# tkoolen/Parametron.jl

Hardware: AMD Instinct MI355X
Metric: QP re-evaluations/sec (Q,q,C,d rebuild) at n=4096 (higher is better)
Workload: dtype f64; 1 GPU; C2 dense least-squares QP: n=4096 vars, A 4096x4096, m=512 equality rows, fp64; canonical Q,q,const + C,d MOI triplets; n=4096, r=4096, m=512, objective_mode=canonical, instances_per_gpu=1, parallelism=single GPU, replay=tape

## Files before the change

parametron.jl_amd/csrc/gram_mid.hip:

```cpp
#include "gram_common.h"

#ifndef PMT_MID_WPS
#define PMT_MID_WPS 1
#endif
#ifndef PMT_MID_G
#define PMT_MID_G 256
#endif
#ifndef PMT_MID_MAXWG
#define PMT_MID_MAXWG 2304
#endif
#ifndef PMT_MID_D
#define PMT_MID_D 2
#endif
#ifndef PMT_MID_GROUP_US
#define PMT_MID_GROUP_US 1.15
#endif
#ifndef PMT_MID_TAIL_US
#define PMT_MID_TAIL_US 0.95
#endif
#ifndef PMT_MID_XCD
#define PMT_MID_XCD 1
#endif
#ifndef PMT_MID_SUPER
#define PMT_MID_SUPER 1
#endif
#ifndef PMT_MID_PERSIST
#define PMT_MID_PERSIST 1
#endif
#ifndef PMT_MID_SB
#define PMT_MID_SB 8
#endif
#ifndef PMT_MID_FB
#define PMT_MID_FB 4
#endif
#ifndef PMT_MID_SCHED
#define PMT_MID_SCHED 2
#endif
#ifndef PMT_MID_ABL
#define PMT_MID_ABL 0
#endif
#ifndef PMT_MID_FORMAL
#if defined(__HIP_DEVICE_COMPILE__) && !defined(__gfx950__) && !defined(__gfx942__)
#define PMT_MID_FORMAL 1
#else
#define PMT_MID_FORMAL 0
#endif
#endif

#ifdef PMT_MID_TRACE
__device__ unsigned long long g_mid_trace[1024 * 8];
#define MID_STAMP(k) do { if (threadIdx.x == 0 && blockIdx.x < 1024) g_mid_trace[blockIdx.x * 8 + (k)] = wall_clock64(); } while (0)
extern "C" int pmt_mid_trace_read(unsigned long long *host) {
    return hipMemcpyFromSymbol(host, HIP_SYMBOL(g_mid_trace), sizeof(unsigned long long) * 1024 * 8) == hipSuccess ? 0 : 1;
}
#else
#define MID_STAMP(k) do { } while (0)
#endif

namespace pmt {

constexpr int MT = 64;
constexpr int MACC = 64;
constexpr int MPART = MACC * 64;
constexpr int MSTRIDE = MPART + MT + 8;
constexpr int MPITCH = MT + 1;
constexpr int MFG = 8;
constexpr int MCNT = 16;
constexpr int MQBUF = 4 * 2048;
constexpr int MFLAG = MQBUF + 4 * MT;
constexpr int MMAPS = MFLAG + 8;
constexpr int MSH = MMAPS + 2 * MT;

struct MidArgs {
    const double *A; int64_t lda, rows, cols;
    const double *b; int sign;
    const int64_t *xvar; const int64_t *varmap; int moi;
    QT *out_quad; double *out_csc; double alpha; LT *out_lin; double *out_const;
    int nb;
    int n_off, s_off, s_diag;
    int gpc_off, gpc_diag;
    int n_tail, s_tail, gpc_tail;
    double *ws;
    unsigned *counters;
    int xcd;
    int persist, total;
    unsigned *tickets;
};

struct MidPlan { int nb, n_off, s_off, s_diag, gpc_off, gpc_diag, n_tail, s_tail, gpc_tail, wgs; };

static double mid_fold_us(int count) { return 0.5 + 2.6 * (double)cdiv(count, PMT_MID_FB); }

static MidPlan mid_plan(int64_t rows, int64_t cols) {
    MidPlan p;
    p.nb = (int)cdiv(cols, MT);
    p.n_off = p.nb * (p.nb - 1) / 2;
    const int ngroups = (int)std::max<int64_t>(1, cdiv(rows, 8));
    const int maxs = std::max(1, ngroups / 4);
    auto sd = [&](int s) { return std::min(maxs, std::max(1, (5 * s + 7) / 8)); };
    int best = 1;
    double best_t = 1e300;
    for (int s = 1; s <= std::min(maxs, 64); ++s) {
        const int64_t wgs = (int64_t)p.n_off * s + (int64_t)p.nb * sd(s);
        if (s > 1 && wgs > PMT_MID_MAXWG) break;
        const double it_off = (double)cdiv(cdiv(ngroups, s), 4), it_diag = 0.69 * (double)cdiv(cdiv(ngroups, sd(s)), 4);
        const double fold = s <= 1 ? 0.0 : s <= MFG ? mid_fold_us(s) : mid_fold_us(MFG) + 1.5 + mid_fold_us((int)cdiv(s, MFG));
        const double t = (double)cdiv(wgs, PMT_MID_G) * (PMT_MID_GROUP_US * (p.n_off ? std::max(it_off, it_diag) : it_diag) + 5.0 + (s > 1 ? 1.0 : 0.0)) +
                         fold * (1.0 + (double)(p.n_off + p.nb) / PMT_MID_G);
        if (t < best_t) { best_t = t; best = s; }
    }
    int s = best;
#ifdef PMT_TUNING
    if (const char *e = getenv("PMT_MID_S")) { const int v = atoi(e); if (v > 0) s = std::min(v, maxs); }
#endif
    int sdiag = sd(s), ntail = 0, stail = 1;
    if (p.n_off + p.nb > PMT_MID_G) {
        auto wg_us = [&](int c, double w) { return PMT_MID_TAIL_US * w * (double)cdiv(cdiv(ngroups, c), 4) + 5.0 + (c > 1 ? 1.0 : 0.0); };
        const int rem = p.n_off % PMT_MID_G;
        int ct = 1;
        double tail_off = 0.0;
        if (rem) {
            tail_off = 1e300;
            for (int c = 1; c <= std::min(maxs, MFG); ++c) {
                const double t = (double)cdiv((int64_t)rem * c, PMT_MID_G) * wg_us(c, 1.0) + (c > 1 ? mid_fold_us(c) : 0.0);
                if (t < tail_off) { tail_off = t; ct = c; }
            }
        }
        const int last = rem ? (int)(((int64_t)rem * ct) % PMT_MID_G) : 0, free_cus = last ? PMT_MID_G - last : 0;
        const double t_last = rem ? wg_us(ct, 1.0) : wg_us(1, 1.0);
        int cd = 1;
        double tail_diag = 1e300;
        for (int c = 1; c <= std::min(maxs, MFG); ++c) {
            const double t_d = wg_us(c, 0.69);
            const int64_t inside = (int64_t)free_cus * (int64_t)(t_last / t_d);
            const int64_t left = std::max<int64_t>(0, (int64_t)p.nb * c - inside);
            const double t = (double)cdiv(left, PMT_MID_G) * t_d + (c > 1 ? mid_fold_us(c) : 0.0);
            if (t < tail_diag) { tail_diag = t; cd = c; }
        }
        const double t1 = (double)(p.n_off / PMT_MID_G) * wg_us(1, 1.0) + tail_off + tail_diag;
        if (s == 1 || t1 * (PMT_MID_GROUP_US / PMT_MID_TAIL_US) < best_t) { s = 1; sdiag = cd; ntail = ct > 1 ? rem : 0; stail = ct > 1 ? ct : 1; }
    }
#ifdef PMT_TUNING
    if (const char *e = getenv("PMT_MID_TAIL")) { if (atoi(e) == 0) { ntail = 0; stail = 1; } }
#endif
    p.gpc_off = (int)cdiv(ngroups, s);
    p.s_off = (int)cdiv(ngroups, p.gpc_off);
    p.gpc_diag = (int)cdiv(ngroups, sdiag);
    p.s_diag = (int)cdiv(ngroups, p.gpc_diag);
    p.n_tail = ntail;
    p.gpc_tail = (int)cdiv(ngroups, stail);
    p.s_tail = ntail ? (int)cdiv(ngroups, p.gpc_tail) : 1;
    if (p.s_tail <= 1) { p.n_tail = 0; p.s_tail = 1; p.gpc_tail = ngroups; }
    p.wgs = (p.n_off - p.n_tail) * p.s_off + p.n_tail * p.s_tail + p.nb * p.s_diag + 1;
    return p;
}

template <bool DIAG, bool FAST>
__device__ __forceinline__ void mid_load(const MidArgs &g, int64_t row0, int lane, int64_t cj0, int64_t ck0, const unsigned (&voff)[DIAG ? 4 : 8],
                                         f64x2 (&buf)[DIAG ? 4 : 8], f64x2 &cb) {
    constexpr int NG = DIAG ? 4 : 8;
    const int lm = lane & 15, lk = lane >> 4;
    if (FAST) {
        const char *base = reinterpret_cast<const char *>(g.A + row0);
#pragma unroll
        for (int t = 0; t < NG; ++t) buf[t] = *reinterpret_cast<const f64x2 *>(base + voff[t]);
        cb.x = 0.0; cb.y = 0.0;
        if (DIAG && g.b) cb = *reinterpret_cast<const f64x2 *>(g.b + row0 + 2 * lk);
        return;
    }
    const int64_t row = row0 + 2 * lk;
    const bool r0 = row < g.rows, r1 = row + 1 < g.rows;
#pragma unroll
    for (int t = 0; t < NG; ++t) {
        const int64_t col = (t < 4 ? cj0 : ck0) + 16 * (t & 3) + lm;
        const bool cv = col < g.cols;
        const bool v0 = cv && r0, v1 = cv && r1;
        const double *p0 = g.A + (v0 ? col * g.lda + row : 0), *p1 = g.A + (v1 ? col * g.lda + row + 1 : 0);
        const double x = *p0, y = *p1;
        buf[t].x = v0 ? x : 0.0;
        buf[t].y = v1 ? y : 0.0;
    }
    cb.x = 0.0; cb.y = 0.0;
    if (DIAG && g.b) {
        const double x = g.b[r0 ? row : 0], y = g.b[r1 ? row + 1 : 0];
        cb.x = r0 ? x : 0.0;
        cb.y = r1 ? y : 0.0;
    }
}

template <bool DIAG>
__device__ __forceinline__ void mid_compute(double *__restrict__ rot, const f64x2 (&buf)[DIAG ? 4 : 8], const f64x2 &cb, int sign, int lane,
                                            double (&acc)[MACC], double (&qacc)[4]) {
    constexpr int BO = DIAG ? 0 : 4;
    const int lm = lane & 15, lrow = lane & 48;
#pragma unroll
    for (int t = 0; t < (PMT_MID_ABL == 5 || PMT_MID_ABL == 6 ? 0 : 4); ++t) *reinterpret_cast<f64x2 *>(rot + (t * 64 + lane) * 2) = buf[BO + t];
    f64x2 bv[4][4];
#pragma unroll
    for (int c = 0; c < 4; ++c) {
        bv[c][0] = buf[BO + c];
#pragma unroll
        for (int r = 1; r < 4; ++r) {
            if (PMT_MID_ABL == 5 || PMT_MID_ABL == 6) { bv[c][r] = buf[BO + (PMT_MID_ABL == 6 ? 0 : c)]; continue; }
            bv[c][r] = *reinterpret_cast<const f64x2 *>(rot + (c * 64 + lrow + ((lm + 4 * r) & 15)) * 2);
        }
    }
#if PMT_MID_SCHED
    __builtin_amdgcn_sched_barrier(0);
#endif
    constexpr int NC = PMT_MID_ABL == 1 ? 0 : 4;
#pragma unroll
    for (int c = 0; c < NC; ++c)
#pragma unroll
        for (int tm = 0; tm < (DIAG ? c + 1 : 4); ++tm) {
            const int a = (tm * 4 + c) * 4;
            acc[a] = __builtin_amdgcn_mfma_f64_4x4x4f64(buf[tm].x, bv[c][0].x, acc[a], 0, 0, 0);
        }
#pragma unroll
    for (int c = 0; c < NC; ++c)
#pragma unroll
        for (int tm = 0; tm < (DIAG ? c + 1 : 4); ++tm) {
            const int a = (tm * 4 + c) * 4;
            acc[a] = __builtin_amdgcn_mfma_f64_4x4x4f64(buf[tm].y, bv[c][0].y, acc[a], 0, 0, 0);
        }
#if PMT_MID_SCHED
    __builtin_amdgcn_sched_barrier(0);
#endif
#pragma unroll
    for (int c = 0; c < NC; ++c) {
#pragma unroll
        for (int r = 1; r < 4; ++r)
#pragma unroll
            for (int tm = 0; tm < (DIAG ? c + 1 : 4); ++tm) {
                const int a = (tm * 4 + c) * 4 + r;
                acc[a] = __builtin_amdgcn_mfma_f64_4x4x4f64(buf[tm].x, bv[c][r].x, acc[a], 0, 0, 0);
            }
#pragma unroll
        for (int r = 1; r < 4; ++r)
#pragma unroll
            for (int tm = 0; tm < (DIAG ? c + 1 : 4); ++tm) {
                const int a = (tm * 4 + c) * 4 + r;
                acc[a] = __builtin_amdgcn_mfma_f64_4x4x4f64(buf[tm].y, bv[c][r].y, acc[a], 0, 0, 0);
            }
    }
    if (DIAG) {
        const double c0 = signed_const(cb.x, sign), c1 = signed_const(cb.y, sign);
#pragma unroll
        for (int t = 0; t < 4; ++t) qacc[t] = __builtin_amdgcn_mfma_f64_4x4x4f64(buf[t].x, c0, qacc[t], 0, 0, 0);
#pragma unroll
        for (int t = 0; t < 4; ++t) qacc[t] = __builtin_amdgcn_mfma_f64_4x4x4f64(buf[t].y, c1, qacc[t], 0, 0, 0);
    }
}

#define MID_SB() __builtin_amdgcn_sched_barrier(0)
template <bool DIAG>
__device__ __forceinline__ void mid_step(const MidArgs &g, double *__restrict__ rot, int64_t next_row0, unsigned (&voff)[DIAG ? 4 : 8],
                                         f64x2 (&buf)[DIAG ? 4 : 8], f64x2 &cb, int sign, int lane, double (&acc)[MACC], double (&qacc)[4]) {
    constexpr int BO = DIAG ? 0 : 4;
    const int lm = lane & 15, lrow = lane & 48, lk = lane >> 4;
    const char *base = reinterpret_cast<const char *>(g.A + next_row0);
    auto reload = [&](int t) {
        asm volatile("" : "+v"(voff[t]));
        buf[t] = *reinterpret_cast<const f64x2 *>(base + voff[t]);
    };
    f64x2 bv[4][4];
#pragma unroll
    for (int c = 0; c < 4; ++c) bv[c][0] = buf[BO + c];
    auto lds_op = [&](int i) {
        if (i < 4) *reinterpret_cast<f64x2 *>(rot + (i * 64 + lane) * 2) = buf[BO + i];
        else {
            const int c = (i - 4) / 3, r = 1 + (i - 4) % 3;
            bv[c][r] = *reinterpret_cast<const f64x2 *>(rot + (c * 64 + lrow + ((lm + 4 * r) & 15)) * 2);
        }
    };
    MID_SB();
    int k = 0;
#pragma unroll
    for (int pass = 0; pass < 2; ++pass)
#pragma unroll
        for (int c = 0; c < 4; ++c)
#pragma unroll
            for (int tm = 0; tm < (DIAG ? c + 1 : 4); ++tm) {
                const int a = (tm * 4 + c) * 4;
                acc[a] = __builtin_amdgcn_mfma_f64_4x4x4f64(pass ? buf[tm].y : buf[tm].x, pass ? bv[c][0].y : bv[c][0].x, acc[a], 0, 0, 0);
                if (k < 16) { MID_SB(); lds_op(k); MID_SB(); }
                ++k;
            }
    if (DIAG) {
        const double c0 = signed_const(cb.x, sign), c1 = signed_const(cb.y, sign);
#pragma unroll
        for (int t = 0; t < 4; ++t) qacc[t] = __builtin_amdgcn_mfma_f64_4x4x4f64(buf[t].x, c0, qacc[t], 0, 0, 0);
#pragma unroll
        for (int t = 0; t < 4; ++t) qacc[t] = __builtin_amdgcn_mfma_f64_4x4x4f64(buf[t].y, c1, qacc[t], 0, 0, 0);
        MID_SB();
        cb = *reinterpret_cast<const f64x2 *>((g.b ? g.b : g.A) + next_row0 + 2 * lk);
    }
    MID_SB();
    int nb = 0;
#pragma unroll
    for (int tm = 0; tm < 4; ++tm) {
#pragma unroll
        for (int pass = 0; pass < 2; ++pass)
#pragma unroll
            for (int c = (DIAG ? tm : 0); c < 4; ++c)
#pragma unroll
                for (int r = 1; r < 4; ++r) {
                    const int a = (tm * 4 + c) * 4 + r;
                    acc[a] = __builtin_amdgcn_mfma_f64_4x4x4f64(pass ? buf[tm].y : buf[tm].x, pass ? bv[c][r].y : bv[c][r].x, acc[a], 0, 0, 0);
                    if (!DIAG && nb < 4) { MID_SB(); reload(4 + nb); MID_SB(); ++nb; }
                }
        MID_SB();
        reload(tm);
        MID_SB();
    }
}

__host__ __device__ constexpr bool mid_used(bool diag, int a) { return !diag || (a >> 4) <= ((a >> 2) & 3); }

__device__ __forceinline__ void mid_pos(int lane, int a, int &row, int &col) {
    const int i = lane >> 4, b = (lane >> 2) & 3, j = lane & 3;
    row = 16 * (a >> 4) + 4 * b + i;
    col = 16 * ((a >> 2) & 3) + 4 * ((b + (a & 3)) & 3) + j;
}

__device__ __forceinline__ void mid_maps(const MidArgs &g, double *sh, int tid, int jb, int kb) {
    u64 *cmap = reinterpret_cast<u64 *>(sh + MMAPS);
    if (tid >= 2 * MT || (!g.out_quad && jb != kb)) return;
    const int64_t i = (tid < MT ? (int64_t)kb * MT + tid : (int64_t)jb * MT + tid - MT);
    const int64_t v = i < g.cols ? g.xvar[i] : 1;
    cmap[tid] = (u64)(g.moi ? map_var(g.varmap, v) : v);
}

__device__ __forceinline__ void mid_epilogue(const MidArgs &g, double *sh, int tid, int jb, int kb) {
    const int wave = tid >> 6, lane = tid & 63;
    const int64_t n = g.cols, j0 = (int64_t)jb * MT, k0 = (int64_t)kb * MT;
    double *tile = sh;
    const double *qfin = sh + MT * MPITCH;
    const u64 *cmap = reinterpret_cast<const u64 *>(sh + MMAPS);
    const u64 *rmap = cmap + MT;
    if (g.out_csc) {
        const int64_t j = j0 + lane;
#pragma unroll 4
        for (int col = wave; col < MT; col += 4) {
            const int64_t k = k0 + col;
            double c = tile[lane * MPITCH + col];
            if (g.moi || j != k) c = 2 * c;
            if (k < n && j <= k) g.out_csc[k * (k + 1) / 2 + j] = g.alpha * c;
        }
    }
    if (g.out_quad) {
        u64 *out = reinterpret_cast<u64 *>(g.out_quad);
        u64 *desc = reinterpret_cast<u64 *>(sh + MT * MPITCH + MT);
        if (tid < MT) {
            const int64_t j = j0 + tid;
            const int64_t kstart = j > k0 ? j : k0;
            const int64_t kend = (k0 + MT < n) ? k0 + MT : n;
            const int64_t nterms = (j < n && kend > kstart) ? kend - kstart : 0;
            desc[2 * tid] = (u64)(j * n - (j * (j - 1)) / 2 + (kstart - j)) * 3;
            desc[2 * tid + 1] = (u64)nterms | (u64)(kstart - k0) << 16 | (u64)(kstart == j ? 1 : 0) << 24;
        }
        __syncthreads();
        const bool moi = g.moi != 0;
        const int uwave = __builtin_amdgcn_readfirstlane(wave);
#pragma unroll 4
        for (int i = 0; i < MT / 4; ++i) {
            const int row = 4 * i + uwave;
            const u64 w0 = desc[2 * row], info = desc[2 * row + 1];
            const int nterms = (int)(info & 0xffff), coff = (int)((info >> 16) & 0xff);
            const bool dg = ((info >> 24) & 1) != 0;
            double c = tile[row * MPITCH + coff + lane];
            const u64 m = cmap[(coff + lane) & (MT - 1)], rv = rmap[row];
            if (moi || !(dg && lane == 0)) c = 2 * c;
            if (lane < nterms) {
                u64 *d = out + w0 + 3 * lane;
                d[0] = (u64)__double_as_longlong(c);
                d[1] = rv;
                d[2] = m;
            }
        }
    }
    if (jb == kb && tid < MT) {
        const int64_t j = j0 + tid;
        if (j < n) {
            LT t;
            t.coeff = 2 * qfin[tid];
            t.var = (int64_t)rmap[tid];
            g.out_lin[j] = t;
        }
    }
}

__device__ __forceinline__ void mid_constant(const MidArgs &g, double *sh, int tid) {
    const int wave = tid >> 6, lane = tid & 63;
    double s0 = 0.0, s1 = 0.0;
    if (g.b && g.sign) {
        for (int64_t i = tid; i < g.rows; i += 512) { const double c = signed_const(g.b[i], g.sign); s0 = s0 + c * c; }
        for (int64_t i = tid + 256; i < g.rows; i += 512) { const double c = signed_const(g.b[i], g.sign); s1 = s1 + c * c; }
    }
#pragma unroll
    for (int off = 32; off > 0; off >>= 1) { s0 = s0 + __shfl_down(s0, off, 64); s1 = s1 + __shfl_down(s1, off, 64); }
    if (lane == 0) { sh[wave] = s0; sh[4 + wave] = s1; }
    __syncthreads();
    if (tid == 0) {
        double v = sh[0];
#pragma unroll
        for (int w = 1; w < 8; ++w) v = v + sh[w];
        *g.out_const = v;
    }
}

__device__ __forceinline__ void mid_put(double *p, double v) {
#if PMT_MID_FORMAL
    *p = v;
#else
    __hip_atomic_store(p, v, __ATOMIC_RELAXED, __HIP_MEMORY_SCOPE_AGENT);
#endif
}
__device__ __forceinline__ double mid_get(const double *p) {
#if PMT_MID_FORMAL
    return *p;
#else
    return __hip_atomic_load(p, __ATOMIC_RELAXED, __HIP_MEMORY_SCOPE_AGENT);
#endif
}

template <bool DIAG, int W>
__device__ __forceinline__ void mid_tail(const MidArgs &g, double *sh, int lane, double (&acc)[MACC], const double (&qacc)[4], int nchunk, double *w) {
    constexpr int KEEP1 = (W >> 1) * 32, GIVE1 = 32 - KEEP1, KEEP2 = KEEP1 + (W & 1) * 16, GIVE2 = KEEP1 + 16 - (W & 1) * 16;
    double *mine = sh + W * 2048;
    const double *half = sh + (W ^ 2) * 2048, *quarter = sh + (W ^ 1) * 2048;
    const bool qlane = (lane & 3) == 0;
    const int qcol = 4 * ((lane >> 2) & 3) + (lane >> 4);
#pragma unroll
    for (int a = 0; a < 32; a += 2)
        if (mid_used(DIAG, GIVE1 + a)) { f64x2 v; v.x = acc[GIVE1 + a]; v.y = acc[GIVE1 + a + 1]; *reinterpret_cast<f64x2 *>(mine + (a * 32 + lane) * 2) = v; }
    if (DIAG && qlane) {
#pragma unroll
        for (int t = 0; t < 4; ++t) sh[MQBUF + W * MT + 16 * t + qcol] = qacc[t];
    }
    __syncthreads();
#pragma unroll
    for (int a = 0; a < 32; a += 2)
        if (mid_used(DIAG, KEEP1 + a)) {
            const f64x2 v = *reinterpret_cast<const f64x2 *>(half + (a * 32 + lane) * 2);
            acc[KEEP1 + a] = acc[KEEP1 + a] + v.x; acc[KEEP1 + a + 1] = acc[KEEP1 + a + 1] + v.y;
        }
    double qsum = 0.0;
    if (DIAG && W == 0) qsum = (sh[MQBUF + lane] + sh[MQBUF + 2 * MT + lane]) + (sh[MQBUF + MT + lane] + sh[MQBUF + 3 * MT + lane]);
    __syncthreads();
#pragma unroll
    for (int a = 0; a < 16; a += 2)
        if (mid_used(DIAG, GIVE2 + a)) { f64x2 v; v.x = acc[GIVE2 + a]; v.y = acc[GIVE2 + a + 1]; *reinterpret_cast<f64x2 *>(mine + (a * 32 + lane) * 2) = v; }
    __syncthreads();
#pragma unroll
    for (int a = 0; a < 16; a += 2)
        if (mid_used(DIAG, KEEP2 + a)) {
            const f64x2 v = *reinterpret_cast<const f64x2 *>(quarter + (a * 32 + lane) * 2);
            acc[KEEP2 + a] = acc[KEEP2 + a] + v.x; acc[KEEP2 + a + 1] = acc[KEEP2 + a + 1] + v.y;
        }
    __syncthreads();
    if (nchunk == 1) {
#pragma unroll
        for (int a = KEEP2; a < KEEP2 + 16; ++a) {
            if (!mid_used(DIAG, a)) continue;
            int row, col;
            mid_pos(lane, a, row, col);
            sh[row * MPITCH + col] = acc[a];
        }
        if (DIAG && W == 0) sh[MT * MPITCH + lane] = qsum;
        return;
    }
#pragma unroll
    for (int a = KEEP2; a < KEEP2 + 16; ++a) if (mid_used(DIAG, a)) mid_put(&w[a * 64 + lane], acc[a]);
    if (DIAG && W == 0) mid_put(&w[MPART + lane], qsum);
#if PMT_MID_FORMAL
    __builtin_amdgcn_fence(__ATOMIC_RELEASE, "agent");
#else
    __builtin_amdgcn_s_waitcnt(0);
#endif
}

template <bool DIAG>
__device__ __forceinline__ void mid_fold(const double *p, int count, int64_t stride, int tid, double (&sum)[16], double &qs) {
#pragma unroll
    for (int u = 0; u < 16; ++u) sum[u] = 0.0;
    qs = 0.0;
    for (int c0 = 0; c0 < count; c0 += PMT_MID_FB) {
        double v[PMT_MID_FB][16], qv[PMT_MID_FB];
#pragma unroll
        for (int cc = 0; cc < PMT_MID_FB; ++cc) {
            const double *pc = p + (int64_t)min(c0 + cc, count - 1) * stride;
#pragma unroll
            for (int u = 0; u < 16; ++u) {
                const int a = (tid >> 6) + 4 * u;
                v[cc][u] = 0.0;
                if (mid_used(DIAG, a)) v[cc][u] = mid_get(pc + tid + 256 * u);
            }
            qv[cc] = 0.0;
            if (DIAG && tid < MT) qv[cc] = mid_get(pc + MPART + tid);
        }
#pragma unroll
        for (int cc = 0; cc < PMT_MID_FB; ++cc) {
            const bool live = c0 + cc < count;
#pragma unroll
            for (int u = 0; u < 16; ++u) { const double t = sum[u] + v[cc][u]; sum[u] = live ? t : sum[u]; }
            const double t = qs + qv[cc];
            qs = live ? t : qs;
        }
    }
}

template <bool DIAG, bool FAST>
__device__ __forceinline__ void mid_body(const MidArgs &g, double *sh, int tid, int jb, int kb, int chunk, int nchunk, int gpc, int first_wg, unsigned *counter) {
    constexpr int NG = DIAG ? 4 : 8;
    constexpr int D = PMT_MID_D;
    const int lane = tid & 63;
    const int wave = __builtin_amdgcn_readfirstlane(tid >> 6);
    const int lm = lane & 15, lk = lane >> 4;
    const int64_t cj0 = (int64_t)jb * MT, ck0 = (int64_t)kb * MT;
    const int ngroups = (int)((g.rows + 7) >> 3);
    const int g0 = chunk * gpc + wave, g1 = min((chunk + 1) * gpc, ngroups);
    const int my = g1 > g0 ? (g1 - g0 + 3) / 4 : 0;
    const bool ragged = FAST && (g.rows & 7) && my > 0 && g0 + 4 * (my - 1) == ngroups - 1;
    const int nfast = ragged ? my - 1 : my;

    MID_STAMP(0);
    mid_maps(g, sh, tid, jb, kb);
    double acc[MACC], qacc[4] = {0.0, 0.0, 0.0, 0.0};
#pragma unroll
    for (int a = 0; a < MACC; ++a) acc[a] = 0.0;
    unsigned voff[NG];
#pragma unroll
    for (int t = 0; t < NG; ++t) voff[t] = (unsigned)((min((t < 4 ? cj0 : ck0) + 16 * (t & 3) + lm, g.cols - 1) * g.lda + 2 * lk) * 8);
    double *rot = sh + wave * 512;
    f64x2 buf[D][NG], cb[D];
    auto row_of = [&](int s) { return (int64_t)(g0 + 4 * min(s, max(nfast - 1, 0))) * 8; };
    if (nfast > 0) {
#pragma unroll
        for (int d = 0; d < D; ++d) mid_load<DIAG, FAST>(g, row_of(d), lane, cj0, ck0, voff, buf[d], cb[d]);
        if (PMT_MID_SCHED == 2 && FAST && PMT_MID_ABL == 0) {
            int s0 = 0;
            for (; s0 + D <= nfast; s0 += D) {
#pragma unroll
                for (int d = 0; d < D; ++d) mid_step<DIAG>(g, rot, row_of(s0 + d + D), voff, buf[d], cb[d], g.sign, lane, acc, qacc);
            }
#pragma unroll
            for (int d = 0; d < D - 1; ++d)
                if (s0 + d < nfast) mid_compute<DIAG>(rot, buf[d], cb[d], g.sign, lane, acc, qacc);
        } else {
            for (int s0 = 0; s0 < nfast; s0 += D) {
#pragma unroll
                for (int d = 0; d < D; ++d) {
                    if (s0 + d < nfast) mid_compute<DIAG>(rot, buf[d], cb[d], g.sign, lane, acc, qacc);
                    if (PMT_MID_ABL != 2) mid_load<DIAG, FAST>(g, row_of(s0 + d + D), lane, cj0, ck0, voff, buf[d], cb[d]);
                }
            }
        }
    }
    if (ragged) {
        mid_load<DIAG, false>(g, (int64_t)(ngroups - 1) * 8, lane, cj0, ck0, voff, buf[0], cb[0]);
        mid_compute<DIAG>(rot, buf[0], cb[0], g.sign, lane, acc, qacc);
    }

    MID_STAMP(1);
    unsigned *flag = reinterpret_cast<unsigned *>(sh + MFLAG);
    double *w = g.ws + (int64_t)(first_wg + chunk) * MSTRIDE;
    __syncthreads();
    if (wave == 0) mid_tail<DIAG, 0>(g, sh, lane, acc, qacc, nchunk, w);
    else if (wave == 1) mid_tail<DIAG, 1>(g, sh, lane, acc, qacc, nchunk, w);
    else if (wave == 2) mid_tail<DIAG, 2>(g, sh, lane, acc, qacc, nchunk, w);
    else mid_tail<DIAG, 3>(g, sh, lane, acc, qacc, nchunk, w);
    MID_STAMP(2);
    if (nchunk > 1) {
        const bool two = nchunk > MFG;
        const int gfirst = two ? (chunk / MFG) * MFG : 0;
        const int n1 = two ? min(MFG, nchunk - gfirst) : nchunk;
        unsigned *c1 = two ? counter + 1 + chunk / MFG : counter;
        __syncthreads();
        if (tid == 0) *flag = __hip_atomic_fetch_add(c1, 1u, __ATOMIC_RELAXED, __HIP_MEMORY_SCOPE_AGENT);
        __syncthreads();
        MID_STAMP(3);
        if (PMT_MID_ABL == 3 || *flag != (unsigned)(n1 - 1)) return;
#if PMT_MID_FORMAL
        __builtin_amdgcn_fence(__ATOMIC_ACQUIRE, "agent");
#endif
        if (tid == 0) __hip_atomic_store(c1, 0u, __ATOMIC_RELAXED, __HIP_MEMORY_SCOPE_AGENT);
        double sum[16], qs;
        double *p = g.ws + (int64_t)(first_wg + gfirst) * MSTRIDE;
        mid_fold<DIAG>(p, n1, MSTRIDE, tid, sum, qs);
        if (two) {
#pragma unroll
            for (int u = 0; u < 16; ++u) if (mid_used(DIAG, (tid >> 6) + 4 * u)) mid_put(p + tid + 256 * u, sum[u]);
            if (DIAG && tid < MT) mid_put(p + MPART + tid, qs);
#if PMT_MID_FORMAL
            __builtin_amdgcn_fence(__ATOMIC_RELEASE, "agent");
#else
            __builtin_amdgcn_s_waitcnt(0);
#endif
            __syncthreads();
            if (tid == 0) *flag = __hip_atomic_fetch_add(counter, 1u, __ATOMIC_RELAXED, __HIP_MEMORY_SCOPE_AGENT);
            __syncthreads();
            const int ng = (nchunk + MFG - 1) / MFG;
            if (*flag != (unsigned)(ng - 1)) return;
#if PMT_MID_FORMAL
            __builtin_amdgcn_fence(__ATOMIC_ACQUIRE, "agent");
#endif
            if (tid == 0) __hip_atomic_store(counter, 0u, __ATOMIC_RELAXED, __HIP_MEMORY_SCOPE_AGENT);
            mid_fold<DIAG>(g.ws + (int64_t)first_wg * MSTRIDE, ng, (int64_t)MFG * MSTRIDE, tid, sum, qs);
        }
        __syncthreads();
        MID_STAMP(4);
#pragma unroll
        for (int u = 0; u < 16; ++u) {
            const int a = (tid >> 6) + 4 * u;
            if (!mid_used(DIAG, a)) continue;
            int row, col;
            mid_pos(lane, a, row, col);
            sh[row * MPITCH + col] = sum[u];
        }
        if (DIAG && tid < MT) sh[MT * MPITCH + tid] = qs;
    }
    __syncthreads();
    MID_STAMP(5);
    if (PMT_MID_ABL != 4) mid_epilogue(g, sh, tid, jb, kb);
#ifdef PMT_MID_TRACE
    __builtin_amdgcn_s_waitcnt(0);
    MID_STAMP(6);
#endif
}

__device__ __forceinline__ int mid_xcd_rank(int id, int base, int n) {
    const int x = id & 7, end = base + n;
    int start = 0;
    for (int y = 0; y < x; ++y) {
        const int fy = base + ((y - base) & 7);
        start += fy < end ? ((end - 1 - fy) >> 3) + 1 : 0;
    }
    return start + ((id - (base + ((x - base) & 7))) >> 3);
}

__device__ __forceinline__ void mid_tile_of(int t, int nb, int &jb, int &kb) {
    constexpr int SB = PMT_MID_SB;
    const int nsb = (nb + SB - 1) / SB;
    for (int K = 0; K < nsb; ++K) {
        const int wK = min(SB, nb - SB * K);
        for (int J = 0; J <= K; ++J) {
            const int cnt = J < K ? SB * wK : wK * (wK - 1) / 2;
            if (t >= cnt) { t -= cnt; continue; }
            if (J < K) { jb = SB * J + t / wK; kb = SB * K + t % wK; return; }
            int kk = 1;
            while (t >= kk) { t -= kk; ++kk; }
            jb = SB * K + t; kb = SB * K + kk;
            return;
        }
    }
    jb = 0; kb = 1;
}

template <bool FAST>
__device__ __forceinline__ void mid_item(const MidArgs &g, double *sh, int tid, int id) {
    const int nbody = g.n_off - g.n_tail, wbody = nbody * g.s_off, noff = wbody + g.n_tail * g.s_tail;
    if (id < noff) {
        const bool tail = id >= wbody;
        const int base = tail ? wbody : 0, ntile = tail ? g.n_tail : nbody, nch = tail ? g.s_tail : g.s_off;
        const int k = g.xcd ? mid_xcd_rank(id, base, ntile * nch) : ((id - base) % nch) * ntile + (id - base) / nch;
        const int chunk = k / ntile;
        const int rank = (tail ? nbody : 0) + (k - chunk * ntile);
        int t = rank, jb, kb;
        if (PMT_MID_SUPER && g.xcd) mid_tile_of(t, g.nb, jb, kb);
        else {
            kb = 1;
            while (t >= kb) { t -= kb; ++kb; }
            jb = t;
        }
        const int first = tail ? wbody + (rank - nbody) * g.s_tail : rank * g.s_off;
        mid_body<false, FAST>(g, sh, tid, jb, kb, chunk, nch, tail ? g.gpc_tail : g.gpc_off, first, g.counters + rank * MCNT);
        return;
    }
    if (id < noff + g.nb * g.s_diag) {
        const int k = g.xcd ? mid_xcd_rank(id, noff, g.nb * g.s_diag) : ((id - noff) % g.s_diag) * g.nb + (id - noff) / g.s_diag;
        const int chunk = k / g.nb, jb = k - chunk * g.nb;
        mid_body<true, FAST>(g, sh, tid, jb, jb, chunk, g.s_diag, g.gpc_diag, noff + jb * g.s_diag, g.counters + (g.n_off + jb) * MCNT);
        return;
    }
    mid_constant(g, sh, tid);
}

template <bool FAST>
__global__ __launch_bounds__(256, PMT_MID_WPS) void gram_mid_kernel(MidArgs g) {
    __shared__ double sh[MSH];
    __shared__ int next_id;
    const int tid = threadIdx.x;
    const int x = blockIdx.x & 7, per = gridDim.x >> 3;
    int id = blockIdx.x;
    for (;;) {
        mid_item<FAST>(g, sh, tid, id);
        if (!g.persist) return;
        __syncthreads();
        if (tid == 0) next_id = x + 8 * (per + (int)__hip_atomic_fetch_add(g.tickets + x, 1u, __ATOMIC_RELAXED, __HIP_MEMORY_SCOPE_AGENT));
        __syncthreads();
        id = next_id;
        if (id >= g.total) break;
    }
    if (tid == 0) {
        const unsigned gone = __hip_atomic_fetch_add(g.tickets + 8, 1u, __ATOMIC_RELAXED, __HIP_MEMORY_SCOPE_AGENT);
        if (gone == gridDim.x - 1) {
#pragma unroll
            for (int i = 0; i < 9; ++i) __hip_atomic_store(g.tickets + i, 0u, __ATOMIC_RELAXED, __HIP_MEMORY_SCOPE_AGENT);
        }
    }
}

__global__ __launch_bounds__(256) void gram_mid_constant_kernel(MidArgs g) {
    __shared__ double sh[8];
    mid_constant(g, sh, threadIdx.x);
}
int launch_gram_mid_constant(const double *b, int sign, int64_t rows, double *out_const, hipStream_t s) {
    MidArgs g = {};
    g.rows = rows; g.b = (b && sign) ? b : nullptr; g.sign = g.b ? sign : 0; g.out_const = out_const;
    PMT_LAUNCH_NAMED("gram_mid_constant_kernel", gram_mid_constant_kernel, dim3(1), dim3(256), 0, s, g);
    return check_launch("gram_mid_constant_kernel");
}

size_t gram_mid_workspace_bytes(int64_t rows, int64_t cols) {
    if (cols <= 0) return 0;
    const MidPlan p = mid_plan(rows, cols);
    return sizeof(double) * (size_t)p.wgs * MSTRIDE;
}
int gram_mid_counters(int64_t cols) { const int nb = (int)cdiv(cols, MT); return MCNT * (nb * (nb + 1) / 2) + 16; }

int launch_gram_mid(const double *A, int64_t lda, int64_t rows, int64_t cols, const int64_t *xvar, const double *b, int sign, int moi,
                    const int64_t *varmap, pmt_quadratic_term *out_quad, double *out_csc, double alpha, pmt_linear_term *out_lin,
                    double *out_const, void *workspace, unsigned *counters, hipStream_t s) {
    if (!workspace || !counters) return fail(PMT_INVALID_ARGUMENT, "quad_gram: workspace required");
    const MidPlan p = mid_plan(rows, cols);
    MidArgs g;
    g.A = A; g.lda = lda; g.rows = rows; g.cols = cols; g.b = (b && sign) ? b : nullptr; g.sign = g.b ? sign : 0;
    g.xvar = xvar; g.varmap = varmap; g.moi = moi; g.out_quad = reinterpret_cast<QT *>(out_quad); g.out_csc = out_csc; g.alpha = alpha;
    g.out_lin = reinterpret_cast<LT *>(out_lin); g.out_const = out_const;
    g.nb = p.nb; g.n_off = p.n_off; g.s_off = p.s_off; g.s_diag = p.s_diag; g.gpc_off = p.gpc_off; g.gpc_diag = p.gpc_diag;
    g.n_tail = p.n_tail; g.s_tail = p.s_tail; g.gpc_tail = p.gpc_tail;
    g.ws = reinterpret_cast<double *>(workspace); g.counters = counters;
    g.xcd = PMT_MID_XCD && rows * cols * 8 > ((int64_t)4 << 20);
    const bool fast = (reinterpret_cast<uintptr_t>(A) & 15) == 0 && (lda & 1) == 0 && (reinterpret_cast<uintptr_t>(g.b) & 15) == 0 &&
                      (uint64_t)lda * (uint64_t)cols * 8 < (1ull << 32);
    g.total = p.wgs;
    g.persist = PMT_MID_PERSIST && p.wgs >= 2 * PMT_MID_G;
    g.tickets = counters + gram_mid_counters(cols) - 16;
    const unsigned grid = g.persist ? (unsigned)PMT_MID_G : (unsigned)p.wgs;
    if (fast) PMT_LAUNCH_NAMED("gram_mid_kernel", (gram_mid_kernel<true>), dim3(grid), dim3(256), 0, s, g);
    else PMT_LAUNCH_NAMED("gram_mid_kernel", (gram_mid_kernel<false>), dim3(grid), dim3(256), 0, s, g);
    return check_launch("gram_mid_kernel");
}

}
```

Before: 892.5 re-evaluations/s.

## Add 128x128 quad-tile work items with simulated scheduling for Gram kernel

Adds a new work-item type in which one 256-thread workgroup computes a 2x2 block of 64x64 Gram tiles over all rows. Each wave handles one sub-tile, which is meant to cut the per-tile overhead of split-K partial sums and fold passes for most off-diagonal tiles. The leftover off-diagonal and diagonal tiles still use the existing path. A host-side list-scheduling simulator picks between the old plan and the quad plan, and plans are cached per shape. The trade-off is more per-thread accumulation work over the full row range, plus host planning cost and complexity on the first call.

```diff
diff --git a/parametron.jl_amd/csrc/gram_mid.hip b/parametron.jl_amd/csrc/gram_mid.hip
--- a/parametron.jl_amd/csrc/gram_mid.hip
+++ b/parametron.jl_amd/csrc/gram_mid.hip
@@ -1,4 +1,9 @@
 #include "gram_common.h"
+
+#include <map>
+#include <mutex>
+#include <queue>
+#include <vector>
 
 #ifndef PMT_MID_WPS
 #define PMT_MID_WPS 1
@@ -35,6 +40,18 @@
 #endif
 #ifndef PMT_MID_SCHED
 #define PMT_MID_SCHED 2
+#endif
+#ifndef PMT_MID_QUAD
+#define PMT_MID_QUAD 1
+#endif
+#ifndef PMT_MID_QSB
+#define PMT_MID_QSB 4
+#endif
+#ifndef PMT_MID_QBAR
+#define PMT_MID_QBAR 0
+#endif
+#ifndef PMT_MID_QUAD_US
+#define PMT_MID_QUAD_US 12.0
 #endif
 #ifndef PMT_MID_ABL
 #define PMT_MID_ABL 0
@@ -69,7 +86,9 @@
 constexpr int MQBUF = 4 * 2048;
 constexpr int MFLAG = MQBUF + 4 * MT;
 constexpr int MMAPS = MFLAG + 8;
-constexpr int MSH = MMAPS + 2 * MT;
+constexpr int MSH64 = MMAPS + 2 * MT;
+constexpr int MQT = MT * MPITCH;
+constexpr int MSH = MSH64 > 4 * MQT ? MSH64 : 4 * MQT;
 
 struct MidArgs {
     const double *A; int64_t lda, rows, cols;
@@ -85,14 +104,26 @@
     int xcd;
     int persist, total;
     unsigned *tickets;
+    int nquad, nqp;
 };
 
-struct MidPlan { int nb, n_off, s_off, s_diag, gpc_off, gpc_diag, n_tail, s_tail, gpc_tail, wgs; };
+struct MidPlan { int nb, n_off, s_off, s_diag, gpc_off, gpc_diag, n_tail, s_tail, gpc_tail, wgs, nquad, nqp; };
+
+__host__ __device__ __forceinline__ int mid_xcd_rank(int id, int base, int n) {
+    const int x = id & 7, end = base + n;
+    int start = 0;
+    for (int y = 0; y < x; ++y) {
+        const int fy = base + ((y - base) & 7);
+        start += fy < end ? ((end - 1 - fy) >> 3) + 1 : 0;
+    }
+    return start + ((id - (base + ((x - base) & 7))) >> 3);
+}
 
 static double mid_fold_us(int count) { return 0.5 + 2.6 * (double)cdiv(count, PMT_MID_FB); }
 
-static MidPlan mid_plan(int64_t rows, int64_t cols) {
+static MidPlan mid_plan64(int64_t rows, int64_t cols) {
     MidPlan p;
+    p.nquad = 0; p.nqp = 0;
     p.nb = (int)cdiv(cols, MT);
     p.n_off = p.nb * (p.nb - 1) / 2;
     const int ngroups = (int)std::max<int64_t>(1, cdiv(rows, 8));
@@ -152,6 +183,82 @@
     p.s_tail = ntail ? (int)cdiv(ngroups, p.gpc_tail) : 1;
     if (p.s_tail <= 1) { p.n_tail = 0; p.s_tail = 1; p.gpc_tail = ngroups; }
     p.wgs = (p.n_off - p.n_tail) * p.s_off + p.n_tail * p.s_tail + p.nb * p.s_diag + 1;
+    return p;
+}
+
+static double mid_sim(const MidPlan &p, int64_t rows) {
+    const int ngroups = (int)std::max<int64_t>(1, cdiv(rows, 8));
+    const int nbody = p.n_off - p.n_tail, wbody = nbody * p.s_off, noff = wbody + p.n_tail * p.s_tail, ndiag = p.nb * p.s_diag;
+    auto chunk_us = [&](int gpc, int s, int chunk, double w) {
+        return PMT_MID_TAIL_US * w * (double)cdiv(gpc, 4) + 5.0 + (s > 1 ? 1.0 : 0.0) + (s > 1 && chunk == s - 1 ? mid_fold_us(s) : 0.0);
+    };
+    auto item_us = [&](int id) {
+        if (id < p.nquad) return PMT_MID_TAIL_US * (double)ngroups + PMT_MID_QUAD_US;
+        const int q0 = p.nquad, r = id - q0;
+        if (r < noff) {
+            const bool tail = r >= wbody;
+            const int base = tail ? wbody : 0, ntile = tail ? p.n_tail : nbody, nch = tail ? p.s_tail : p.s_off;
+            return chunk_us(tail ? p.gpc_tail : p.gpc_off, nch, mid_xcd_rank(id, q0 + base, ntile * nch) / ntile, 1.0);
+        }
+        if (r < noff + ndiag) return chunk_us(p.gpc_diag, p.s_diag, mid_xcd_rank(id, q0 + noff, ndiag) / p.nb, 0.69);
+        return 2.0;
+    };
+    double end = 0.0;
+    for (int x = 0; x < 8; ++x) {
+        std::priority_queue<double, std::vector<double>, std::greater<double>> free_at;
+        for (int i = 0; i < PMT_MID_G / 8; ++i) free_at.push(0.0);
+        for (int id = x; id < p.wgs; id += 8) {
+            const double t = free_at.top() + item_us(id);
+            free_at.pop();
+            free_at.push(t);
+            end = std::max(end, t);
+        }
+    }
+    return end;
+}
+
+static MidPlan mid_plan_quad(int64_t rows, const MidPlan &b, double &best_t) {
+    const int ngroups = (int)std::max<int64_t>(1, cdiv(rows, 8));
+    const int maxs = std::min(MFG, std::max(1, ngroups / 4));
+    MidPlan p = b, best = b;
+    p.nqp = p.nb / 2;
+    p.nquad = p.nqp * (p.nqp - 1) / 2;
+    p.n_off = p.nqp + ((p.nb & 1) ? p.nb - 1 : 0);
+    p.s_off = 1;
+    p.gpc_off = ngroups;
+    best_t = 1e300;
+    for (int c = 1; c <= maxs; ++c)
+        for (int cd = 1; cd <= maxs; ++cd) {
+            p.gpc_tail = (int)cdiv(ngroups, c);
+            p.s_tail = (int)cdiv(ngroups, p.gpc_tail);
+            p.n_tail = p.s_tail > 1 ? p.n_off : 0;
+            if (!p.n_tail) { p.s_tail = 1; p.gpc_tail = ngroups; }
+            p.gpc_diag = (int)cdiv(ngroups, cd);
+            p.s_diag = (int)cdiv(ngroups, p.gpc_diag);
+            p.wgs = p.nquad + (p.n_off - p.n_tail) * p.s_off + p.n_tail * p.s_tail + p.nb * p.s_diag + 1;
+            const double t = mid_sim(p, rows);
+            if (t < best_t) { best_t = t; best = p; }
+        }
+    return best;
+}
+
+static MidPlan mid_plan(int64_t rows, int64_t cols) {
+    static std::mutex mu;
+    static std::map<std::pair<int64_t, int64_t>, MidPlan> known;
+    {
+        std::lock_guard<std::mutex> lock(mu);
+        auto it = known.find({rows, cols});
+        if (it != known.end()) return it->second;
+    }
+    MidPlan p = mid_plan64(rows, cols);
+    if (PMT_MID_QUAD && p.nb >= 4 && p.wgs >= 2 * PMT_MID_G) {
+        double tq;
+        const MidPlan q = mid_plan_quad(rows, p, tq);
+        if (tq < mid_sim(p, rows)) p = q;
+    }
+    std::lock_guard<std::mutex> lock(mu);
+    if (known.size() >= 256) known.clear();
+    known[{rows, cols}] = p;
     return p;
 }
 
@@ -629,18 +736,7 @@
 #endif
 }
 
-__device__ __forceinline__ int mid_xcd_rank(int id, int base, int n) {
-    const int x = id & 7, end = base + n;
-    int start = 0;
-    for (int y = 0; y < x; ++y) {
-        const int fy = base + ((y - base) & 7);
-        start += fy < end ? ((end - 1 - fy) >> 3) + 1 : 0;
-    }
-    return start + ((id - (base + ((x - base) & 7))) >> 3);
-}
-
-__device__ __forceinline__ void mid_tile_of(int t, int nb, int &jb, int &kb) {
-    constexpr int SB = PMT_MID_SB;
+__device__ __forceinline__ void mid_tile_of(int t, int nb, int SB, int &jb, int &kb) {
     const int nsb = (nb + SB - 1) / SB;
     for (int K = 0; K < nsb; ++K) {
         const int wK = min(SB, nb - SB * K);
@@ -657,17 +753,134 @@
     jb = 0; kb = 1;
 }
 
+__device__ __forceinline__ void mid_left_of(int r, int nqp, int nb, int &jb, int &kb) {
+    if (r < nqp) { jb = 2 * r; kb = 2 * r + 1; }
+    else { jb = r - nqp; kb = nb - 1; }
+}
+
+template <bool FAST>
+__device__ __forceinline__ void mid_quad(const MidArgs &g, double *sh, int tid, int J, int K) {
+    constexpr int NG = 8;
+    constexpr int D = PMT_MID_D;
+    const int lane = tid & 63;
+    const int wave = __builtin_amdgcn_readfirstlane(tid >> 6);
+    const int lm = lane & 15, lk = lane >> 4;
+    const int jb = 2 * J + (wave >> 1), kb = 2 * K + (wave & 1);
+    const int64_t n = g.cols, cj0 = (int64_t)jb * MT, ck0 = (int64_t)kb * MT;
+    const int ngroups = (int)((g.rows + 7) >> 3);
+    const bool ragged = FAST && (g.rows & 7);
+    const int nfast = ragged ? ngroups - 1 : ngroups;
+
+    MID_STAMP(0);
+    u64 cm = 0, rm = 0;
+    if (g.out_quad) {
+        const int64_t vc = ck0 + lane < n ? g.xvar[ck0 + lane] : 1, vr = cj0 + lane < n ? g.xvar[cj0 + lane] : 1;
+        cm = (u64)(g.moi ? map_var(g.varmap, vc) : vc);
+        rm = (u64)(g.moi ? map_var(g.varmap, vr) : vr);
+    }
+    double acc[MACC], qacc[4] = {0.0, 0.0, 0.0, 0.0};
+#pragma unroll
+    for (int a = 0; a < MACC; ++a) acc[a] = 0.0;
+    unsigned voff[NG];
+#pragma unroll
+    for (int t = 0; t < NG; ++t) voff[t] = (unsigned)((min((t < 4 ? cj0 : ck0) + 16 * (t & 3) + lm, g.cols - 1) * g.lda + 2 * lk) * 8);
+    double *rot = sh + wave * 512;
+    f64x2 buf[D][NG], cb[D];
+    auto row_of = [&](int s) { return (int64_t)min(s, max(nfast - 1, 0)) * 8; };
+    if (nfast > 0) {
+#pragma unroll
+        for (int d = 0; d < D; ++d) mid_load<false, FAST>(g, row_of(d), lane, cj0, ck0, voff, buf[d], cb[d]);
+        if (PMT_MID_SCHED == 2 && FAST && PMT_MID_ABL == 0) {
+            int s0 = 0;
+            for (; s0 + D <= nfast; s0 += D) {
+                if (PMT_MID_QBAR > 0 && s0 % (D * (PMT_MID_QBAR > 0 ? PMT_MID_QBAR : 1)) == 0) __builtin_amdgcn_s_barrier();
+#pragma unroll
+                for (int d = 0; d < D; ++d) mid_step<false>(g, rot, row_of(s0 + d + D), voff, buf[d], cb[d], g.sign, lane, acc, qacc);
+            }
+#pragma unroll
+            for (int d = 0; d < D - 1; ++d)
+                if (s0 + d < nfast) mid_compute<false>(rot, buf[d], cb[d], g.sign, lane, acc, qacc);
+        } else {
+            for (int s0 = 0; s0 < nfast; s0 += D) {
+#pragma unroll
+                for (int d = 0; d < D; ++d) {
+                    if (s0 + d < nfast) mid_compute<false>(rot, buf[d], cb[d], g.sign, lane, acc, qacc);
+                    if (PMT_MID_ABL != 2) mid_load<false, FAST>(g, row_of(s0 + d + D), lane, cj0, ck0, voff, buf[d], cb[d]);
+                }
+            }
+        }
+    }
+    if (ragged) {
+        mid_load<false, false>(g, (int64_t)(ngroups - 1) * 8, lane, cj0, ck0, voff, buf[0], cb[0]);
+        mid_compute<false>(rot, buf[0], cb[0], g.sign, lane, acc, qacc);
+    }
+    MID_STAMP(1);
+    __syncthreads();
+    double *tile = sh + wave * MQT;
+#pragma unroll
+    for (int a = 0; a < MACC; ++a) {
+        int row, col;
+        mid_pos(lane, a, row, col);
+        tile[row * MPITCH + col] = acc[a];
+    }
+    __syncthreads();
+    MID_STAMP(5);
+    if (PMT_MID_ABL == 4) return;
+    if (g.out_csc) {
+        const int64_t j = cj0 + lane;
+#pragma unroll 4
+        for (int col = 0; col < MT; ++col) {
+            const int64_t k = ck0 + col;
+            const double c = 2 * tile[lane * MPITCH + col];
+            if (k < n && j <= k) g.out_csc[k * (k + 1) / 2 + j] = g.alpha * c;
+        }
+    }
+    if (g.out_quad) {
+        u64 *out = reinterpret_cast<u64 *>(g.out_quad);
+        const int nterms = (int)(min(ck0 + MT, n) - ck0);
+        const int rows = (int)min((int64_t)MT, n - cj0);
+        for (int row = 0; row < rows; ++row) {
+            const int64_t j = cj0 + row;
+            const u64 w0 = (u64)(j * n - (j * (j - 1)) / 2 + (ck0 - j)) * 3;
+            const double c = 2 * tile[row * MPITCH + lane];
+            const u64 rv = (u64)(unsigned)__builtin_amdgcn_readlane((int)(unsigned)rm, row) |
+                           (u64)(unsigned)__builtin_amdgcn_readlane((int)(unsigned)(rm >> 32), row) << 32;
+            if (lane < nterms) {
+                u64 *d = out + w0 + 3 * lane;
+                d[0] = (u64)__double_as_longlong(c);
+                d[1] = rv;
+                d[2] = cm;
+            }
+        }
+    }
+#ifdef PMT_MID_TRACE
+    __builtin_amdgcn_s_waitcnt(0);
+    MID_STAMP(6);
+#endif
+}
+
 template <bool FAST>
 __device__ __forceinline__ void mid_item(const MidArgs &g, double *sh, int tid, int id) {
+    if (id < g.nquad) {
+        const int k = g.xcd ? mid_xcd_rank(id, 0, g.nquad) : id;
+        int J, K;
+        mid_tile_of(k, g.nqp, PMT_MID_QSB, J, K);
+        mid_quad<FAST>(g, sh, tid, J, K);
+        return;
+    }
+    const int q0 = g.nquad;
     const int nbody = g.n_off - g.n_tail, wbody = nbody * g.s_off, noff = wbody + g.n_tail * g.s_tail;
+    const int id0 = id;
+    id -= q0;
     if (id < noff) {
         const bool tail = id >= wbody;
         const int base = tail ? wbody : 0, ntile = tail ? g.n_tail : nbody, nch = tail ? g.s_tail : g.s_off;
-        const int k = g.xcd ? mid_xcd_rank(id, base, ntile * nch) : ((id - base) % nch) * ntile + (id - base) / nch;
+        const int k = g.xcd ? mid_xcd_rank(id0, q0 + base, ntile * nch) : ((id - base) % nch) * ntile + (id - base) / nch;
         const int chunk = k / ntile;
         const int rank = (tail ? nbody : 0) + (k - chunk * ntile);
         int t = rank, jb, kb;
-        if (PMT_MID_SUPER && g.xcd) mid_tile_of(t, g.nb, jb, kb);
+        if (g.nquad) mid_left_of(t, g.nqp, g.nb, jb, kb);
+        else if (PMT_MID_SUPER && g.xcd) mid_tile_of(t, g.nb, PMT_MID_SB, jb, kb);
         else {
             kb = 1;
             while (t >= kb) { t -= kb; ++kb; }
@@ -678,7 +891,7 @@
         return;
     }
     if (id < noff + g.nb * g.s_diag) {
-        const int k = g.xcd ? mid_xcd_rank(id, noff, g.nb * g.s_diag) : ((id - noff) % g.s_diag) * g.nb + (id - noff) / g.s_diag;
+        const int k = g.xcd ? mid_xcd_rank(id0, q0 + noff, g.nb * g.s_diag) : ((id - noff) % g.s_diag) * g.nb + (id - noff) / g.s_diag;
         const int chunk = k / g.nb, jb = k - chunk * g.nb;
         mid_body<true, FAST>(g, sh, tid, jb, jb, chunk, g.s_diag, g.gpc_diag, noff + jb * g.s_diag, g.counters + (g.n_off + jb) * MCNT);
         return;
@@ -725,7 +938,7 @@
 size_t gram_mid_workspace_bytes(int64_t rows, int64_t cols) {
     if (cols <= 0) return 0;
     const MidPlan p = mid_plan(rows, cols);
-    return sizeof(double) * (size_t)p.wgs * MSTRIDE;
+    return sizeof(double) * (size_t)(p.wgs - p.nquad) * MSTRIDE;
 }
 int gram_mid_counters(int64_t cols) { const int nb = (int)cdiv(cols, MT); return MCNT * (nb * (nb + 1) / 2) + 16; }
 
@@ -740,12 +953,13 @@
     g.out_lin = reinterpret_cast<LT *>(out_lin); g.out_const = out_const;
     g.nb = p.nb; g.n_off = p.n_off; g.s_off = p.s_off; g.s_diag = p.s_diag; g.gpc_off = p.gpc_off; g.gpc_diag = p.gpc_diag;
     g.n_tail = p.n_tail; g.s_tail = p.s_tail; g.gpc_tail = p.gpc_tail;
+    g.nquad = p.nquad; g.nqp = p.nqp;
     g.ws = reinterpret_cast<double *>(workspace); g.counters = counters;
     g.xcd = PMT_MID_XCD && rows * cols * 8 > ((int64_t)4 << 20);
     const bool fast = (reinterpret_cast<uintptr_t>(A) & 15) == 0 && (lda & 1) == 0 && (reinterpret_cast<uintptr_t>(g.b) & 15) == 0 &&
                       (uint64_t)lda * (uint64_t)cols * 8 < (1ull << 32);
     g.total = p.wgs;
-    g.persist = PMT_MID_PERSIST && p.wgs >= 2 * PMT_MID_G;
+    g.persist = PMT_MID_PERSIST && (p.wgs >= 2 * PMT_MID_G || (p.nquad && p.wgs > PMT_MID_G));
     g.tickets = counters + gram_mid_counters(cols) - 16;
     const unsigned grid = g.persist ? (unsigned)PMT_MID_G : (unsigned)p.wgs;
     if (fast) PMT_LAUNCH_NAMED("gram_mid_kernel", (gram_mid_kernel<true>), dim3(grid), dim3(256), 0, s, g);
```

After: 920.5 re-evaluations/s, median of 6. 1.03x the previous value.
